# Suaiba/Mammo-CLIP-Dissect

Hardware: AMD Instinct MI355X
Metric: probe images/sec dissected (763 concepts, all layers) (higher is better)
Workload: dtype f32; 1 GPU; configs[1]: M-Mammo-CLIP Dissect through the drop-in driver describe_broad_neurons.main(): Mammo-CLIP ViT-B/16 target+dissector (random init), weak: 10000 images per GPU, synthetic 224x224 images resident in HBM, 763 concepts, 12 layers x 768 neurons, soft_wpmi top_k=100; CSV + args.txt + activation cache files written inside the step; entry_point=mammo_clip_dissect_amd.concept_vit.describe_broad_neurons.main, images_per_gpu=10000, global_images=10000, batch=2500, parallelism=image-sharded dp1, activation_cache_written=True

## Files before the change

### mammo-clip-dissect_amd/_lib.py

```python
import ctypes
import os

_HERE = os.path.dirname(os.path.abspath(__file__))
LIB_PATH = os.environ.get("MCD_LIB_PATH") or os.path.join(_HERE, "csrc", "libmcd_hip.so")

_i64 = ctypes.c_int64
_int = ctypes.c_int
_f = ctypes.c_float
_p = ctypes.c_void_p
_sz = ctypes.c_size_t

SIGNATURES = {
    "mcd_last_error": (ctypes.c_char_p, []),
    "mcd_abi_version": (_int, []),
    "mcd_normalize_rows": (_int, [_p, _i64, _i64, _i64, _p, _i64, _p]),
    "mcd_center_cube_normalize_rows": (_int, [_p, _i64, _i64, _i64, _f, _p, _i64, _p]),
    "mcd_prepare_rows_gathered": (_int, [_p, _i64, _i64, _int, ctypes.POINTER(_i64), _i64, _i64, _i64, _int, _f, _p, _i64,
                                         _p]),
    "mcd_embed_gemm_workspace": (_sz, [_i64, _i64, _i64, _int]),
    "mcd_embed_gemm": (_int, [_p, _i64, _p, _i64, _i64, _i64, _i64, _int, _p, _i64, _p, _sz, _p]),
    "mcd_embed_gemm_exp_workspace": (_sz, [_i64, _i64, _i64]),
    "mcd_embed_gemm_exp": (_int, [_p, _i64, _p, _i64, _i64, _i64, _i64, _f, _int, _p, _i64, _p, _p, _sz, _p]),
    "mcd_embed_gemm_exp_time_kernel": (_int, [_int]),
    "mcd_embed_gemm_exp_kernel_ms": (_f, []),
# ... 9 lines not shown
    "mcd_row_topk": (_int, [_p, _i64, _i64, _i64, _int, _p, _p, _p]),
    "mcd_hook_pool": (_int, [_p, _i64, _i64, _i64, _int, _p, _i64, _i64, _i64, _i64, _p]),
    "mcd_rank_reorder": (_int, [_p, _i64, _i64, _i64, _p, _p, _i64, _i64, _int, _p, _int, _f, _f, _p, _p, _i64, _p]),
    "mcd_vit_attention": (_int, [_p, _i64, _i64, _i64, _p, _p]),
    "mcd_vit_attention_long": (_int, [_p, _i64, _i64, _i64, _p, _p]),
    "mcd_vit_attention_cls": (_int, [_p, _i64, _p, _i64, _i64, _p, _i64, _i64, _i64, _i64, _i64, _p, _p]),
    "mcd_layer_norm": (_int, [_p, _i64, _i64, _p, _p, _f, _p, _p]),
    "mcd_patchify": (_int, [_p, _i64, _i64, _i64, _i64, _i64, _p, _p]),
    "mcd_conv_stem_nhwc": (_int, [_p, _i64, _i64, _i64, _i64, _p, _p, _i64, _p, _p]),
    "mcd_dwconv_bn_silu": (_int, [_p, _i64, _i64, _i64, _i64, _p, _p, _int, _int, _int, _p, _p, _i64, _p]),
    "mcd_se_gate": (_int, [_p, _i64, _i64, _i64, _i64, _p, _p, _i64, _p, _p, _p, _p]),
    "mcd_channel_scale": (_int, [_p, _i64, _i64, _i64, _p, _p]),
    "mcd_hook_pool_nhwc": (_int, [_p, _i64, _i64, _i64, _int, _p, _i64, _i64, _i64, _i64, _p]),
    "mcd_conv7x7s2_nhwc": (_int, [_p, _i64, _i64, _i64, _i64, _p, _i64, _p, _p]),
    "mcd_bn_relu_maxpool_nhwc": (_int, [_p, _i64, _i64, _i64, _i64, _p, _p, _p, _p]),
    "mcd_conv_igemm_nhwc": (_int, [_p, _i64, _i64, _i64, _i64, _p, _p, _i64, _int, _int, _int, _int, _p, _p]),
    "mcd_conv_igemm_res_nhwc": (_int, [_p, _i64, _i64, _i64, _i64, _p, _p, _p, _i64, _int, _int, _int, _int, _p, _p]),
    "mcd_conv3x3s2_nhwc": (_int, [_p, _i64, _i64, _i64, _i64, _p, _p, _i64, _int, _p, _p]),
    "mcd_avgpool2_nhwc": (_int, [_p, _i64, _i64, _i64, _i64, _p, _p]),
    "mcd_attnpool_tokens": (_int, [_p, _i64, _i64, _i64, _p, _p, _p]),
    "mcd_image_preprocess": (_int, [_p, _i64, _i64, _i64, _p, _i64, _i64, _p, _i64, _i64, _i64, _i64, _i64, _i64, _p, _p, _i64,
                                    _p]),
    "mcd_image_minmax_workspace": (_sz, [_i64, _i64, _i64, _i64]),
    "mcd_image_minmax_normalize": (_int, [_p, _i64, _i64, _i64, _i64, _int, _f, _f, _p, _i64, _p, _sz, _p]),
}
TEXT_SIGNATURES = {
    "mcd_vit_attention_keylen": (_int, [_p, _i64, _i64, _i64, _p, _p, _p]),
    "mcd_text_embed_ln": (_int, [_p, _p, _p, _p, _p, _p, _p, _f, _i64, _i64, _i64, _i64, _i64, _p, _p]),
}
CLIP_SIGNATURES = {
    "mcd_vit_attention_causal": (_int, [_p, _i64, _i64, _i64, _p, _p]),
    "mcd_quick_gelu": (_int, [_p, _i64, _p, _p]),
}
TOKEN_SIGNATURES = {
    "mcd_token_mean": (_int, [_p, _int, _int, _int, _i64, _i64, _int, _p, _i64, _p]),
}
SENTENCE_SIGNATURES = {
    "mcd_vit_attention_relbias": (_int, [_p, _i64, _i64, _i64, _p, _p, _p, _p]),
    "mcd_masked_mean_l2": (_int, [_p, _int, _int, _int, _p, _int, _p, _p]),
}
MASK_SIGNATURES = {
    "mcd_patchify_kept": (_int, [_p, _p, _i64, _i64, _i64, _i64, _i64, _i64, _p, _p]),
    "mcd_token_restore": (_int, [_p, _i64, _p, _p, _p, _i64, _i64, _i64, _i64, _p, _p]),
}
_pp = ctypes.POINTER(_p)
CACHE_SIGNATURES = {
    "mcd_hook_pool_rows": (_int, [_p, _i64, _i64, _i64, _int, _p, _i64, _i64, _i64, _i64, _p, _i64, _p]),
    "mcd_cache_stream_open": (_int, [_int, _pp, ctypes.POINTER(_i64), _p, _int, _sz, _pp]),
    "mcd_cache_stream_reserve": (_int, [_p, _int, _p]),
    "mcd_cache_stream_push": (_int, [_p, _int, _p, _i64, _i64, _p]),
    "mcd_cache_stream_close": (_int, [_p]),
    "mcd_cache_stream_abort": (_int, [_p]),
}

MCD_E_ARG = -1
MCD_E_RANGE = -2
MCD_E_WORKSPACE = -3
MCD_E_UNSUPPORTED = -5

_lib = None


class McdError(RuntimeError):

    def __init__(self, code, msg):
        super().__init__(msg)
        self.code = code


def load():
    global _lib
    if _lib is None:
        if not os.path.exists(LIB_PATH):
            raise ImportError(
                "mammo-clip-dissect_amd: %s not found. Build it with `python -c 'import __graft_entry__ as g; "
                "g.build()'` or `make -C mammo-clip-dissect_amd/csrc`. There is no CPU fallback." % LIB_PATH)
        L = ctypes.CDLL(LIB_PATH)
        for name, (res, args) in (list(SIGNATURES.items()) + list(TEXT_SIGNATURES.items()) + list(CLIP_SIGNATURES.items())
                                  + list(TOKEN_SIGNATURES.items()) + list(SENTENCE_SIGNATURES.items())
                                  + list(MASK_SIGNATURES.items()) + list(CACHE_SIGNATURES.items())):
            fn = getattr(L, name)
            fn.restype = res
            fn.argtypes = args
        _lib = L
    return _lib


def check(rc):
    if rc != 0:
        msg = load().mcd_last_error().decode("utf-8", "replace")
        raise McdError(rc, msg)


BLASLT_PATH = os.path.join(os.path.dirname(LIB_PATH), "libmcd_blaslt.so")
BLASLT_SIGNATURES = {
    "mcd_blaslt_last_error": (ctypes.c_char_p, []),
    "mcd_linear_residual_workspace": (_sz, []),
    "mcd_linear_residual": (_int, [_p, _i64, _p, _i64, _p, _p, _i64, _p, _i64, _i64, _i64, _i64, _p, _sz, _p]),
    "mcd_linear_residual_relu": (_int, [_p, _i64, _p, _i64, _p, _p, _i64, _p, _i64, _i64, _i64, _i64, _p, _sz, _p]),
    "mcd_linear_residual_plan_info": (_int, [_i64, _i64, _i64, ctypes.POINTER(_f), ctypes.POINTER(_int)]),
    "mcd_linear_residual_get_picks": (_int, [ctypes.POINTER(_i64), _int]),
    "mcd_linear_residual_set_pick": (_int, [_i64, _i64, _i64, _int, _int]),
}
_blaslt = None


def load_blaslt():
    global _blaslt
    if _blaslt is None:
        try:
            L = ctypes.CDLL(BLASLT_PATH)
            for name, (res, args) in BLASLT_SIGNATURES.items():
                fn = getattr(L, name)
                fn.restype = res
                fn.argtypes = args
            _blaslt = L
        except (OSError, AttributeError):
            _blaslt = False
    return _blaslt or None


HOST_PATH = os.path.join(_HERE, "csrc", "libmcd_host.so")
CACHE_HOST_SIGNATURES = {
    "mcd_zip_crc32": (ctypes.c_uint32, [ctypes.c_uint32, _p, _sz]),
    "mcd_cachefile_open": (_int, [ctypes.c_char_p, ctypes.c_char_p, _i64, _i64, _i64, _i64, _i64, _pp]),
    "mcd_cachefile_append": (_int, [_p, _p, _i64, _i64]),
    "mcd_cachefile_close": (_int, [_p]),
    "mcd_cachefile_abort": (None, [_p]),
    "mcd_cachefile_last_error": (ctypes.c_char_p, []),
}
_cache_host = None


# ... 22 lines not shown
```

### mammo-clip-dissect_amd/concept_vit/data_utils.py

```python
import collections
import math
import os
import unicodedata
import zlib

import torch
import torch.nn as nn
import torch.nn.functional as F
from torch.nn.modules import module as _nn_module

from .. import core

PROJ_DIM = 512
HIP_ATTENTION = os.environ.get("MCD_NO_HIP_ATTENTION", "0") != "1"
ATTENTION_EVENTS = None
_attention_calls = 0
FUSED_RESIDUAL = os.environ.get("MCD_NO_FUSED_RESIDUAL", "0") != "1"
CLS_ONLY_TAIL = os.environ.get("MCD_NO_CLS_ONLY_TAIL", "0") != "1"


HIP_LAYER_NORM = os.environ.get("MCD_NO_HIP_LAYER_NORM", "0") != "1"
HIP_MBCONV = os.environ.get("MCD_NO_HIP_MBCONV", "0") != "1"
HIP_RESNET = os.environ.get("MCD_NO_HIP_RESNET", "0") != "1"
HIP_CLIP_RN = os.environ.get("MCD_NO_HIP_CLIP_RN", "0") != "1"
HIP_TEXT = os.environ.get("MCD_NO_HIP_TEXT", "0") != "1"
HIP_CLIP_TEXT = os.environ.get("MCD_NO_HIP_CLIP_TEXT", "0") != "1"
MAX_BATCH = 65535


def _hip_eligible(on_gpu, dtype, grad):
    return bool(on_gpu) and dtype == torch.float32 and not grad


def _eligible(x):
    return isinstance(x, torch.Tensor) and _hip_eligible(x.is_cuda, x.dtype, torch.is_grad_enabled())


def _tower_gate(flag, module, x):
    return bool(flag and _eligible(x) and x.dim() == 4 and not module.training and x.shape[0] <= MAX_BATCH
                and core.linear_residual_available())


def _under_2g(*elements):
    return all(n * 4 < 2 ** 31 for n in elements)


class _LayerNorm(nn.LayerNorm):

    def forward(self, x):
        D = x.shape[-1]
        if (HIP_LAYER_NORM and _eligible(x) and x.is_contiguous() and len(self.normalized_shape) == 1 and D % 4 == 0
                and D <= 2048 and self.weight is not None and self.bias is not None):
            return core.layer_norm(x, self.weight, self.bias, self.eps)
        return super().forward(x)


def _linear(mod, x):
    if _fused_residual_ok(x) and x.is_contiguous() and mod.bias is not None:
        return core.linear_residual(None, x, mod.weight, mod.bias)
    return mod(x)


def _fused_residual_ok(x):
    return bool(FUSED_RESIDUAL and _eligible(x) and core.linear_residual_available())


def attention_route(T, D, heads, masked, on_gpu, dtype, needs_grad):
    if not (HIP_ATTENTION and not masked and _hip_eligible(on_gpu, dtype, needs_grad) and D == 64 * heads):
        return "sdpa"
    if T <= core.VIT_ATTENTION_MAX_T:
        return "k9"
    if T <= core.VIT_ATTENTION_LONG_MAX_T and _under_2g(T * 3 * D):
        return "long"
    return "sdpa"


def cls_tail_route(flag, fused_ok, masked, training, T, D, heads, depth, hooks_clear, last_hooks_token0):
    return bool(flag and HIP_ATTENTION and fused_ok and not masked and not training and D == 64 * heads
                and 1 <= T <= core.VIT_ATTENTION_CLS_MAX_T and depth >= 1 and hooks_clear and last_hooks_token0)


def embed_gate(P, H, W, table_rows):
    return bool(P >= 2 and P % 2 == 0 and H % P == 0 and W % P == 0 and 1 + (H // P) * (W // P) == table_rows)


def _token0_hooks(m):
    return all(getattr(h, "token0_only", False) for h in m._forward_hooks.values())


def _cls_tail_ok(x, blocks, container, clear=(), token0=()):
    if not (CLS_ONLY_TAIL and isinstance(x, torch.Tensor) and x.dim() == 3) or len(blocks) == 0:
        return False
    last = blocks[-1]
    hooks_clear = not (_nn_module._global_forward_hooks or _nn_module._global_forward_pre_hooks or last._forward_pre_hooks
                       or any(_hooked(c) for c in last.children()) or any(_hooked(m) for m in clear)
                       or container._forward_hooks or container._forward_pre_hooks)
    return cls_tail_route(CLS_ONLY_TAIL, _fused_residual_ok(x), False, container.training or last.training, x.shape[1],
                          x.shape[2], last.attn.heads, len(blocks), hooks_clear, all(_token0_hooks(m) for m in (last,) + token0))


def _class_pos_residual(pos, cls, bias, B):
    r = pos.detach().expand(B, -1, -1).contiguous()
    r[:, 0] = cls.detach() + pos.detach()[0] if bias is None else cls.detach() + pos.detach()[0] - bias.detach()
    return r


def _attend(qkv, heads, choice, arg=None):
    B, T, D = qkv.shape[0], qkv.shape[1], qkv.shape[2] // 3
    if choice == "k9":
        global _attention_calls
        _attention_calls += 1
        timed = ATTENTION_EVENTS is not None and _attention_calls % 8 == 0
        if timed:
            e0, e1 = torch.cuda.Event(enable_timing=True), torch.cuda.Event(enable_timing=True)
            e0.record()
        o = core.vit_attention(qkv, heads)
        if timed:
            e1.record()
            ATTENTION_EVENTS.append((e0, e1, B, T, heads))
        return o
    if choice == "long":
        return core.vit_attention_long(qkv, heads)
    if choice == "causal":
        return core.vit_attention_causal(qkv, heads)
    if choice == "keylen":
        return core.vit_attention_keylen(qkv, heads, arg)
    if choice == "relbias":
        return core.vit_attention_relbias(qkv, heads, *arg)
    q, k, v = qkv.view(B, T, 3, heads, D // heads).permute(2, 0, 3, 1, 4)
    o = F.scaled_dot_product_attention(q, k, v, attn_mask=arg)
    return o.transpose(1, 2).reshape(B, T, D)


def _attend_cls(q, kv):
    return core.vit_attention_cls(q, kv[:, :, 0], kv[:, :, 1])


_BlockOps = collections.namedtuple("_BlockOps", "ln1 ln2 qkv proj fc1 fc2 heads")


def _ln_ops(ln):
    return ln.weight, ln.bias, ln.eps


def _lin_ops(lin):
    return lin.weight, lin.bias


def _norm(x, ln, k10=True):
    return core.layer_norm(x, *ln) if k10 else F.layer_norm(x, x.shape[-1:], *ln)


def _gelu(h):
    return F.gelu(h)


def _quick_gelu_(h):
    return core.quick_gelu(h, out=h)


def _block_hip(p, x, attn, attn_arg=None, post=False, act=_gelu, cls_only=False, k10=True):
    B, T, D = x.shape
    x = x.contiguous()
    n = x if post else _norm(x, p.ln1, k10)
    w, b = p.qkv
    if cls_only:
        kv = core.linear_residual(None, n, w[D:], None if b is None else b[D:]).view(B, T, 2, p.heads, D // p.heads)
        o = _attend_cls(core.linear_residual(None, n[:, 0], w[:D], None if b is None else b[:D]), kv)
        x = x[:, 0]
    else:
        o = _attend(core.linear_residual(None, n, w, b), p.heads, attn, attn_arg).contiguous()
    x1 = core.linear_residual(x, o, *p.proj)
    if post:
        x1 = _norm(x1, p.ln1, k10)
    h = act(core.linear_residual(None, x1 if post else _norm(x1, p.ln2, k10), *p.fc1))
    if post:
        return _norm(core.linear_residual(x1, h, *p.fc2), p.ln2, k10)
    out = core.linear_residual(x1, h, *p.fc2, out=x1)
    return out.unsqueeze(1) if cls_only else out


class _Attention(nn.Module):
    def __init__(self, dim, heads):
        super().__init__()
        self.heads = heads
        self.qkv = nn.Linear(dim, 3 * dim)
        self.proj = nn.Linear(dim, dim)

    def forward(self, x, mask=None):
        return self.proj(self.heads_out(x, mask))

    def heads_out(self, x, mask=None):
        qkv = self.qkv(x)
        route = attention_route(x.shape[1], x.shape[2], self.heads, mask is not None, qkv.is_cuda, qkv.dtype,
                                torch.is_grad_enabled() and qkv.requires_grad)
        return _attend(qkv, self.heads, route, mask)


class _LayerScale(nn.Module):

    def __init__(self, dim, init):
        super().__init__()
        self.lambda1 = nn.Parameter(init * torch.ones(dim))

    def forward(self, x):
        return x * self.lambda1


_BLOCK_SKIPPED = ("norm1", "attn", "norm2", "fc1", "fc2", "layer_scale1", "layer_scale2")


class _Block(nn.Module):

    def __init__(self, dim, heads, mlp, eps=1e-12, layer_scale=None):
        super().__init__()
        self.norm1 = _LayerNorm(dim, eps=eps)
        self.attn = _Attention(dim, heads)
        self.norm2 = _LayerNorm(dim, eps=eps)
        self.fc1 = nn.Linear(dim, mlp)
        self.fc2 = nn.Linear(mlp, dim)
        self.scaled = layer_scale is not None
        if self.scaled:
            self.layer_scale1 = _LayerScale(dim, layer_scale)
            self.layer_scale2 = _LayerScale(dim, layer_scale)

    def forward(self, x, mask=None, cls_only=False):
        cls_only = cls_only and mask is None
        if cls_only or (_fused_residual_ok(x) and not _hooks_on(self, _BLOCK_SKIPPED)):
            B, T, D = x.shape
            route = attention_route(T, D, self.attn.heads, mask is not None, x.is_cuda, x.dtype, False)
            return _block_hip(self._ops(), x, route, mask, cls_only=cls_only, k10=HIP_LAYER_NORM and D % 4 == 0 and D <= 2048)
        if self.scaled:
            x = x + self.layer_scale1(self.attn(self.norm1(x), mask))
            return x + self.layer_scale2(self.fc2(F.gelu(self.fc1(self.norm2(x)))))
        x = x + self.attn(self.norm1(x), mask)
        return x + self.fc2(F.gelu(self.fc1(self.norm2(x))))

    def _ops(self):
        wp, bp, w2, b2 = self._residual_weights()
        return _BlockOps(_ln_ops(self.norm1), _ln_ops(self.norm2), _lin_ops(self.attn.qkv), (wp, bp), _lin_ops(self.fc1),
                         (w2, b2), self.attn.heads)

    def _residual_weights(self):
        a = self.attn
        if not self.scaled:
            return a.proj.weight, a.proj.bias, self.fc2.weight, self.fc2.bias

        def build(m):
            l1, l2 = m.layer_scale1.lambda1.detach(), m.layer_scale2.lambda1.detach()
            return ((l1[:, None] * m.attn.proj.weight.detach()).contiguous(), (l1 * m.attn.proj.bias.detach()).contiguous(),
                    (l2[:, None] * m.fc2.weight.detach()).contiguous(), (l2 * m.fc2.bias.detach()).contiguous())
        return _folded(self, ("layer_scale1", "layer_scale2", "attn", "fc2"), build)


class _Encoder(nn.Module):
    def __init__(self, depth, dim, heads, mlp, list_name, eps=1e-12, layer_scale=None):
        super().__init__()
        setattr(self, list_name, nn.ModuleList([_Block(dim, heads, mlp, eps, layer_scale) for _ in range(depth)]))
        self._list_name = list_name

    def forward(self, x, mask=None, cls_only=False):
        blocks = getattr(self, self._list_name)
        for i, blk in enumerate(blocks):
            x = blk(x, mask, cls_only=True) if cls_only and i == len(blocks) - 1 else blk(x, mask)
        return x


def image_hw(image_size):
    if isinstance(image_size, (tuple, list)):
        h, w = image_size
        return int(h), int(w)
    return int(image_size), int(image_size)


def _parse_hw(text):
    if text.isdigit():
        return int(text)
    h, sep, w = text.partition("x")
    if sep and h.isdigit() and w.isdigit():
        return int(h), int(w)
    return None


class ViTTower(nn.Module):

    def __init__(self, image_size=224, patch=16, dim=768, depth=12, heads=12, mlp=3072, list_name="layer", eps=1e-12,
                 layer_scale=None):
        super().__init__()
        self.out_dim = dim
        h, w = image_hw(image_size)
        self._build_embedding(dim, patch, (h // patch) * (w // patch))
        self.encoder = _Encoder(depth, dim, heads, mlp, list_name, eps, layer_scale)
        self.layernorm = _LayerNorm(dim, eps=eps)

# ... 1196 lines not shown
    ok = (flag and _hip_eligible(on_gpu, dtype, grad) and not training and D == 64 * heads and D % 4 == 0 and D <= 2048
          and 1 <= T <= core.VIT_ATTENTION_LONG_MAX_T and _under_2g(T * 3 * D) and 1 <= B <= MAX_BATCH and fused_ok)
    return "hip" if ok else "aten"


def quick_gelu(x):
    return x * torch.sigmoid(1.702 * x)


class _QuickGELU(nn.Module):
    def forward(self, x):
        return quick_gelu(x)


class _ClipMHA(nn.Module):

    def __init__(self, dim, heads):
        super().__init__()
        self.heads = heads
        self.in_proj_weight = nn.Parameter(torch.empty(3 * dim, dim))
        self.in_proj_bias = nn.Parameter(torch.zeros(3 * dim))
        self.out_proj = nn.Linear(dim, dim)

    def forward(self, x, causal=False):
        B, T, D = x.shape
        q, k, v = F.linear(x, self.in_proj_weight, self.in_proj_bias).view(B, T, 3, self.heads, D // self.heads).permute(2, 0, 3, 1, 4)
        o = F.scaled_dot_product_attention(q, k, v, is_causal=causal)
        return self.out_proj(o.transpose(1, 2).reshape(B, T, D))


class _ClipResBlock(nn.Module):

    def __init__(self, dim, heads, causal=False):
        super().__init__()
        self.causal = causal
        self.attn = _ClipMHA(dim, heads)
        self.ln_1 = nn.LayerNorm(dim)
        self.mlp = nn.Sequential()
        self.mlp.add_module("c_fc", nn.Linear(dim, 4 * dim))
        self.mlp.add_module("gelu", _QuickGELU())
        self.mlp.add_module("c_proj", nn.Linear(4 * dim, dim))
        self.ln_2 = nn.LayerNorm(dim)

    def forward(self, x, hip=False, cls_only=False):
        if hip and not _hooks_on(self, _CLIP_BLOCK_SKIPPED):
            attn = "causal" if self.causal else "k9" if x.shape[1] <= core.VIT_ATTENTION_MAX_T else "long"
            return _block_hip(self._ops(), x, attn, act=_quick_gelu_, cls_only=cls_only)
        x = x + self.attn(self.ln_1(x), self.causal)
        return x + self.mlp(self.ln_2(x))

    def _ops(self):
        a, m = self.attn, self.mlp
        return _BlockOps(_ln_ops(self.ln_1), _ln_ops(self.ln_2), (a.in_proj_weight, a.in_proj_bias), _lin_ops(a.out_proj),
                         _lin_ops(m.c_fc), _lin_ops(m.c_proj), a.heads)


class _ClipTransformer(nn.Module):
    def __init__(self, width, layers, heads, causal=False):
        super().__init__()
        self.width, self.layers = width, layers
        self.resblocks = nn.ModuleList([_ClipResBlock(width, heads, causal) for _ in range(layers)])

    def forward(self, x, hip=False, cls_only=False):
        for i, blk in enumerate(self.resblocks):
            x = blk(x, hip, cls_only and i == len(self.resblocks) - 1)
        return x


class _ClipVisionTransformer(nn.Module):

    def __init__(self, input_resolution, patch_size, width, layers, heads, output_dim):
        super().__init__()
        self.input_resolution, self.output_dim = input_resolution, output_dim
        self.conv1 = nn.Conv2d(3, width, patch_size, patch_size, bias=False)
        scale = width ** -0.5
        self.class_embedding = nn.Parameter(scale * torch.randn(width))
        self.positional_embedding = nn.Parameter(scale * torch.randn((input_resolution // patch_size) ** 2 + 1, width))
        self.ln_pre = nn.LayerNorm(width)
        self.transformer = _ClipTransformer(width, layers, heads)
        self.ln_post = nn.LayerNorm(width)
        self.proj = nn.Parameter(scale * torch.randn(width, output_dim))

    def route(self, x):
        P = self.conv1.kernel_size[0]
        n = self.positional_embedding.shape[0]
        heads = self.transformer.resblocks[0].attn.heads if len(self.transformer.resblocks) else 0
        if not (isinstance(x, torch.Tensor) and x.dim() == 4 and x.is_contiguous()
                and embed_gate(P, x.shape[2], x.shape[3], n)):
            return "aten"
        return clip_tower_route(HIP_CLIP_TEXT, x.is_cuda, x.dtype, torch.is_grad_enabled(), self.training, x.shape[0], n,
                                self.conv1.out_channels, heads, _fused_residual_ok(x))

    def forward(self, x):
        x = x.to(self.conv1.weight.dtype)
        if self.route(x) == "hip":
            return self._forward_hip(x)
        x = self.conv1(x).flatten(2).transpose(1, 2)
        x = torch.cat([self.class_embedding.expand(x.shape[0], 1, -1), x], dim=1) + self.positional_embedding
        x = self.transformer(self.ln_pre(x))
        return self.ln_post(x[:, 0]) @ self.proj

    def _forward_hip(self, x):
        B = x.shape[0]
        P = self.conv1.kernel_size[0]
        t = core.linear_residual(self._embed_residual(B), core.patchify(x, P), self.conv1.weight.view(self.conv1.out_channels, -1))
        if _hooked(self.ln_pre) or _nn_module._global_forward_hooks or _nn_module._global_forward_pre_hooks:
            t = self.ln_pre(t)
# ... 1517 lines not shown
```

### mammo-clip-dissect_amd/core.py

```python
import ctypes
import functools

import torch

from . import _lib
from ._lib import McdError, check

POOL_MODES = {"avg": 0, "max": 1, "cls": 2, "none": 3}
POOL_SILU_AVG = 4
GEMM_MODES = {"f32": 0, "bf16x3": 1, "bf16": 2}


def _stream():
    return ctypes.c_void_p(torch.cuda.current_stream().cuda_stream)


def _on_device(fn):
    @functools.wraps(fn)
    def wrapper(*args, **kw):
        dev = None
        for a in list(args) + list(kw.values()):
            if isinstance(a, torch.Tensor) and a.is_cuda:
                if dev is None:
                    dev = a.device
# ... 420 lines not shown
def quick_gelu(x, out=None):
    _need_gpu(x, out)
    if x.dtype != torch.float32 or not x.is_contiguous():
        raise TypeError("x must be a contiguous float32 tensor")
    if out is None:
        out = torch.empty_like(x)
    elif out.dtype != torch.float32 or out.shape != x.shape or not out.is_contiguous():
        raise TypeError("out must be a contiguous float32 tensor of x's shape")
    check(_lib.load().mcd_quick_gelu(x.data_ptr(), x.numel(), out.data_ptr(), _stream()))
    return out


@_on_device
def token_mean(x, t0=1, out=None):
    _need_gpu(x, out)
    if x.dtype != torch.float32 or x.dim() != 3 or x.stride(2) != 1:
        raise TypeError("x must be a float32 [B, T, D] tensor with a unit inner stride")
    B, T, D = x.shape
    if out is None:
        out = torch.empty((B, D), dtype=torch.float32, device=x.device)
    elif out.dtype != torch.float32 or tuple(out.shape) != (B, D) or out.stride(1) != 1:
        raise TypeError("out must be a float32 [B, D] tensor with a unit inner stride")
    check(_lib.load().mcd_token_mean(x.data_ptr(), B, T, D, x.stride(0), x.stride(1), t0, out.data_ptr(), out.stride(0),
                                     _stream()))
    return out


VIT_ATTENTION_CLS_MAX_T = 32768


@_on_device
def vit_attention_cls(q, k, v, out=None):
    _need_gpu(q, k, v, out)
    if any(t.dtype != torch.float32 for t in (q, k, v)) or k.dim() != 4 or k.shape[3] != 64 or v.shape != k.shape:
        raise TypeError("vit_attention_cls: float32 k and v of one shape [B, T, heads, 64]")
    B, T, H, _ = k.shape
    if q.dim() == 3:
        if tuple(q.shape) != (B, H, 64) or (H > 1 and q.stride(1) != 64):
            raise ValueError("vit_attention_cls: q must be [B, heads, 64] with a row's heads adjacent")
    elif tuple(q.shape) != (B, H * 64):
        raise ValueError("vit_attention_cls: q has shape %s, k %s" % (tuple(q.shape), tuple(k.shape)))
    if q.stride(-1) != 1 or any(t.stride(3) != 1 or (H > 1 and t.stride(2) != 64) for t in (k, v)):
        raise ValueError("vit_attention_cls: the heads*64 floats of a token must be adjacent in q, k and v")
    if out is None:
        out = torch.empty((B, H * 64), dtype=torch.float32, device=k.device)
    elif out.dtype != torch.float32 or tuple(out.shape) != (B, H * 64) or not out.is_contiguous():
        raise TypeError("out must be a contiguous float32 [B, heads*64] tensor")
    W = H * 64
    q_img = q.stride(0) if B > 1 else W
    row = [t.stride(1) if T > 1 else W for t in (k, v)]
    img = [t.stride(0) if B > 1 else max(T * r, W) for t, r in zip((k, v), row)]
    check(_lib.load().mcd_vit_attention_cls(q.data_ptr(), q_img, k.data_ptr(), row[0], img[0], v.data_ptr(), row[1], img[1],
                                            B, T, H, out.data_ptr(), _stream()))
    return out


@_on_device
def layer_norm(x, weight, bias, eps):
    _need_gpu(x, weight, bias)
    D = x.shape[-1]
    if x.dtype != torch.float32 or not x.is_contiguous() or weight.shape != (D,) or bias.shape != (D,):
        raise TypeError("layer_norm: contiguous float32 x and [D] weight / bias")
    y = torch.empty_like(x)
    L = _lib.load()
    check(L.mcd_layer_norm(x.data_ptr(), x.numel() // D, D, weight.data_ptr(), bias.data_ptr(), float(eps), y.data_ptr(),
                           _stream()))
    return y


@_on_device
def text_embed_ln(ids, type_ids, word, pos, type_table, weight, bias, eps, out=None):
    _need_gpu(word, pos, type_table, weight, bias, out)
    if ids.dim() != 2 or ids.dtype != torch.int64 or (type_ids is not None and (type_ids.dtype != torch.int64
                                                                               or type_ids.shape != ids.shape)):
        raise TypeError("text_embed_ln: ids (and type_ids) must be int64 [B, T]")
    B, T = ids.shape
    tables = (word, pos, type_table)
    if any(t.dtype != torch.float32 or t.dim() != 2 or not t.is_contiguous() for t in tables):
        raise TypeError("text_embed_ln: contiguous float32 [rows, D] tables")
    D = word.shape[1]
    if pos.shape[1] != D or type_table.shape[1] != D or weight.shape != (D,) or bias.shape != (D,):
        raise ValueError("text_embed_ln: the tables, weight and bias must share the width D=%d" % D)
    if T < 1 or T > pos.shape[0]:
        raise ValueError("text_embed_ln: T=%d tokens, the position table has %d rows" % (T, pos.shape[0]))
    for name, t, n in (("ids", ids, word.shape[0]), ("type_ids", type_ids, type_table.shape[0])):
        if t is not None and not t.is_cuda and t.numel() and (int(t.min()) < 0 or int(t.max()) >= n):
            raise ValueError("text_embed_ln: %s outside [0, %d)" % (name, n))
    ids = ids.to(word.device).contiguous()
    type_ids = None if type_ids is None else type_ids.to(word.device).contiguous()
    if out is None:
        out = torch.empty((B, T, D), dtype=torch.float32, device=word.device)
    elif out.dtype != torch.float32 or tuple(out.shape) != (B, T, D) or not out.is_contiguous():
        raise TypeError("out must be a contiguous float32 [B, T, D] tensor")
    check(_lib.load().mcd_text_embed_ln(ids.data_ptr(), None if type_ids is None else type_ids.data_ptr(), word.data_ptr(),
                                        pos.data_ptr(), type_table.data_ptr(), weight.data_ptr(), bias.data_ptr(), float(eps),
                                        B * T, T, D, word.shape[0], type_table.shape[0], out.data_ptr(), _stream()))
    return out


@_on_device
def patchify(x, patch):
    B, Cin, H, W = _nchw_image(x, "patchify: contiguous float32 [B, Cin, H, W]").shape
    if H % patch or W % patch:
        raise ValueError("patchify: %dx%d is not a multiple of the %d-pixel patch" % (H, W, patch))
    out = torch.empty((B, 1 + (H // patch) * (W // patch), Cin * patch * patch), dtype=torch.float32, device=x.device)
    L = _lib.load()
# ... 255 lines not shown
    if C % 4 or HW < 1:
        raise ValueError("attnpool_tokens: C = %d must be a multiple of 4 and the image non-empty" % C)
    if pos.dtype != torch.float32 or tuple(pos.shape) != (HW + 1, C) or not pos.is_contiguous():
        raise TypeError("attnpool_tokens: pos must be a contiguous float32 [%d, %d] tensor" % (HW + 1, C))
    _aligned16("attnpool_tokens: x and pos must be 16-byte aligned", x, pos)
    tok = torch.empty((B, HW + 1, C), dtype=torch.float32, device=x.device)
    L = _lib.load()
    check(L.mcd_attnpool_tokens(x.data_ptr(), B, HW, C, pos.data_ptr(), tok.data_ptr(), _stream()))
    return tok


_blaslt_ws = {}
LINEAR_EVENTS = None


def linear_residual_available():
    return _lib.load_blaslt() is not None


def encoder_gemm_picks():
    L = _lib.load_blaslt()
    if L is None:
        return []
    n = L.mcd_linear_residual_get_picks(None, 0)
    buf = (ctypes.c_int64 * (5 * max(n, 1)))()
    n = min(n, L.mcd_linear_residual_get_picks(buf, n))
    return [tuple(int(buf[5 * i + j]) for j in range(5)) for i in range(n)]


def set_encoder_gemm_picks(picks):
    L = _lib.load_blaslt()
    if L is None:
        return
    for M, N, K, has_res, pick in picks:
        L.mcd_linear_residual_set_pick(int(M), int(N), int(K), int(has_res), int(pick))


def _row_strided(t):
    return t.dim() == 2 and t.stride(1) == 1 and t.stride(0) >= t.shape[1]


@_on_device
def linear_residual(res, h, weight, bias=None, out=None, relu=False):
    L = _lib.load_blaslt()
    if L is None:
        raise ImportError("libmcd_blaslt.so is not available (make -C mammo-clip-dissect_amd/csrc)")
    _need_gpu(h, weight, bias, res, out)
    K = h.shape[-1]
    N = weight.shape[0]
    if weight.shape[1] != K or (res is not None and (res.shape[-1] != N or res.shape[:-1] != h.shape[:-1])):
        raise ValueError("linear_residual: shapes h %s, weight %s, res %s do not match"
                         % (tuple(h.shape), tuple(weight.shape), None if res is None else tuple(res.shape)))
    for t in (h, weight, bias, res, out):
        if t is not None and (t.dtype != torch.float32 or not (t.is_contiguous() or (t is h or t is res) and _row_strided(t))):
            raise TypeError("linear_residual: contiguous float32 tensors only (h and res: or 2-D row-strided)")
    M = h.numel() // K
    ldh = K if h.is_contiguous() else h.stride(0)
    ldr = N if res is None or res.is_contiguous() else res.stride(0)
    if out is None:
        out = torch.empty(h.shape[:-1] + (N,), dtype=torch.float32, device=h.device)
    elif tuple(out.shape) != tuple(h.shape[:-1]) + (N,):
        raise ValueError("linear_residual: out has shape %s" % (tuple(out.shape),))
    ws = _blaslt_ws.get(h.device)
    if ws is None:
        ws = _blaslt_ws[h.device] = torch.empty((L.mcd_linear_residual_workspace(),), dtype=torch.uint8, device=h.device)
    ev = LINEAR_EVENTS
    if ev is not None:
        e0, e1 = torch.cuda.Event(enable_timing=True), torch.cuda.Event(enable_timing=True)
        e0.record()
    fn = L.mcd_linear_residual_relu if relu else L.mcd_linear_residual
    rc = fn(h.data_ptr(), ldh, weight.data_ptr(), K, bias.data_ptr() if bias is not None else None,
            res.data_ptr() if res is not None else None, ldr, out.data_ptr(), N, M, N, K, ws.data_ptr(), ws.numel(), _stream())
    if ev is not None:
        e1.record()
        ev.append((e0, e1, M, N, K))
    if rc != 0:
        raise _lib.McdError(rc, L.mcd_blaslt_last_error().decode("utf-8", "replace"))
    return out


@_on_device
def hook_pool(x, mode, dst, row0, col0, neuron_major, rows=None):
    _need_gpu(x, dst)
    if rows is not None:
        _need_gpu(rows)
    if x.dtype != torch.float32:
        x = x.float()
    nhwc = mode in ("avg", "max") and channels_last(x, only=True)
    if not nhwc:
        x = x.contiguous()
    if x.dim() == 4:
        B, Cout, HW = x.shape[0], x.shape[1], x.shape[2] * x.shape[3]
        m = POOL_MODES[mode]
    elif x.dim() == 3:
        B, HW, Cout = x.shape
        m = POOL_MODES["cls"]
    elif x.dim() == 2:
        B, Cout = x.shape
        HW = 1
        m = POOL_MODES["none"]
    else:
        raise ValueError("unsupported hook output shape %s" % (tuple(x.shape),))
    if dst.dtype != torch.float32 or dst.dim() != 2 or dst.stride(1) != 1:
        raise TypeError("dst must be a 2-D float32 matrix with unit inner stride")
    need = (col0 + Cout, row0 + B) if neuron_major else (row0 + B, col0 + Cout)
    if row0 < 0 or col0 < 0 or dst.shape[0] < need[0] or dst.shape[1] < need[1]:
        raise IndexError("hook_pool: block [%d:%d, %d:%d] outside the activation matrix %s"
                         % (row0, row0 + B, col0, col0 + Cout, tuple(dst.shape)))
    if neuron_major:
        sn, su = 1, dst.stride(0)
    else:
        sn, su = dst.stride(0), 1
    if rows is not None and (rows.dtype != torch.float32 or rows.dim() != 2 or not rows.is_contiguous()
                             or rows.shape[0] < B or rows.shape[1] != Cout):
        raise TypeError("rows must be a contiguous float32 [>= %d, %d] block" % (B, Cout))
    L = _lib.load()
    if nhwc:
        check(L.mcd_hook_pool_nhwc(x.data_ptr(), B, Cout, HW, m, dst.data_ptr(), int(row0), int(col0), sn, su, _stream()))
        if rows is not None:
            if not neuron_major:
                raise TypeError("hook_pool: rows with a channels-last input needs a neuron-major dst")
            if B > 0:
                transpose(dst[col0:col0 + Cout, row0:row0 + B], out=rows[:B])
        return Cout
    if rows is not None:
# ... 256 lines not shown
```

Measured before the change: 4043 images/s.

## Fold key/value projections into the CLS query for the last-block attention

For the CLS-only tail block, the key weights are folded into the CLS query per head (u = q_h·Wk_h, pre-scaled for exp2). A new HIP kernel computes scores against the normalized tokens, applies softmax and mixes the tokens. The value projection is then applied only to the mixed per-head vectors. This avoids the full B×T K/V projection GEMM of the last layer. In exchange it adds per-head small GEMM launches and a cached folded-weight tensor, and linear_residual now accepts a row-strided output. The key bias is dropped, which is safe because softmax is shift-invariant.

```diff
diff --git a/include/mcd_clsfold.h b/include/mcd_clsfold.h
--- /dev/null
+++ b/include/mcd_clsfold.h
@@ -0,0 +1,18 @@
+#ifndef MCD_CLSFOLD_H
+#define MCD_CLSFOLD_H
+
+#include "mcd_hip.h"
+
+#ifdef __cplusplus
+extern "C" {
+#endif
+
+int mcd_cls_token_mix(const float* u, int64_t u_img, const float* n, int64_t n_row, int64_t n_img, int64_t B, int64_t T,
+                      int64_t H, int64_t D, float* m, int64_t m_img, mcd_stream_t stream);
+
+int64_t mcd_cls_token_mix_max_t(int64_t H, int64_t D);
+
+#ifdef __cplusplus
+}
+#endif
+#endif
diff --git a/mammo-clip-dissect_amd/_lib.py b/mammo-clip-dissect_amd/_lib.py
--- a/mammo-clip-dissect_amd/_lib.py
+++ b/mammo-clip-dissect_amd/_lib.py
@@ -85,6 +85,10 @@
     "mcd_cache_stream_close": (_int, [_p]),
     "mcd_cache_stream_abort": (_int, [_p]),
 }
+CLSFOLD_SIGNATURES = {
+    "mcd_cls_token_mix": (_int, [_p, _i64, _p, _i64, _i64, _i64, _i64, _i64, _i64, _p, _i64, _p]),
+    "mcd_cls_token_mix_max_t": (_i64, [_i64, _i64]),
+}
 
 MCD_E_ARG = -1
 MCD_E_RANGE = -2
@@ -111,7 +115,8 @@
         L = ctypes.CDLL(LIB_PATH)
         for name, (res, args) in (list(SIGNATURES.items()) + list(TEXT_SIGNATURES.items()) + list(CLIP_SIGNATURES.items())
                                   + list(TOKEN_SIGNATURES.items()) + list(SENTENCE_SIGNATURES.items())
-                                  + list(MASK_SIGNATURES.items()) + list(CACHE_SIGNATURES.items())):
+                                  + list(MASK_SIGNATURES.items()) + list(CACHE_SIGNATURES.items())
+                                  + list(CLSFOLD_SIGNATURES.items())):
             fn = getattr(L, name)
             fn.restype = res
             fn.argtypes = args
diff --git a/mammo-clip-dissect_amd/concept_vit/data_utils.py b/mammo-clip-dissect_amd/concept_vit/data_utils.py
--- a/mammo-clip-dissect_amd/concept_vit/data_utils.py
+++ b/mammo-clip-dissect_amd/concept_vit/data_utils.py
@@ -17,6 +17,8 @@
 _attention_calls = 0
 FUSED_RESIDUAL = os.environ.get("MCD_NO_FUSED_RESIDUAL", "0") != "1"
 CLS_ONLY_TAIL = os.environ.get("MCD_NO_CLS_ONLY_TAIL", "0") != "1"
+CLS_FOLD = os.environ.get("MCD_NO_CLS_FOLD", "0") != "1"
+CLS_FOLD_MIN_ROWS = 32768
 
 
 HIP_LAYER_NORM = os.environ.get("MCD_NO_HIP_LAYER_NORM", "0") != "1"
@@ -78,6 +80,11 @@
 def cls_tail_route(flag, fused_ok, masked, training, T, D, heads, depth, hooks_clear, last_hooks_token0):
     return bool(flag and HIP_ATTENTION and fused_ok and not masked and not training and D == 64 * heads
                 and 1 <= T <= core.VIT_ATTENTION_CLS_MAX_T and depth >= 1 and hooks_clear and last_hooks_token0)
+
+
+def cls_fold_route(flag, B, T, D, heads, min_rows):
+    return bool(flag and B * T >= min_rows and D == 64 * heads and D <= 2048 and 1 <= B <= core.CLS_TOKEN_MIX_MAX_B
+                and 1 <= T <= core.cls_token_mix_max_t(heads, D))
 
 
 def embed_gate(P, H, W, table_rows):
@@ -136,7 +143,26 @@
     return core.vit_attention_cls(q, kv[:, :, 0], kv[:, :, 1])
 
 
-_BlockOps = collections.namedtuple("_BlockOps", "ln1 ln2 qkv proj fc1 fc2 heads")
+_LOG2E = 1.4426950408889634
+
+
+def _attend_cls_folded(owner, qkv, heads, q, n):
+    w, b = qkv
+    B, T, D = n.shape
+    wkt = _folded(owner, (), lambda m: (w.detach()[D:2 * D].view(heads, 64, D).transpose(1, 2) * (_LOG2E / 8.0)).contiguous(),
+                  own=True)
+    u = torch.empty((B, heads, D), dtype=n.dtype, device=n.device)
+    for h in range(heads):
+        core.linear_residual(None, q[:, 64 * h:64 * h + 64], wkt[h], None, out=u[:, h])
+    m = core.cls_token_mix(u, n)
+    o = torch.empty((B, D), dtype=n.dtype, device=n.device)
+    for h in range(heads):
+        r = slice(2 * D + 64 * h, 2 * D + 64 * h + 64)
+        core.linear_residual(None, m[:, h], w[r], None if b is None else b[r], out=o[:, 64 * h:64 * h + 64])
+    return o
+
+
+_BlockOps = collections.namedtuple("_BlockOps", "ln1 ln2 qkv proj fc1 fc2 heads owner", defaults=(None,))
 
 
 def _ln_ops(ln):
@@ -164,7 +190,10 @@
     x = x.contiguous()
     n = x if post else _norm(x, p.ln1, k10)
     w, b = p.qkv
-    if cls_only:
+    if cls_only and p.owner is not None and cls_fold_route(CLS_FOLD, B, T, D, p.heads, CLS_FOLD_MIN_ROWS):
+        o = _attend_cls_folded(p.owner, p.qkv, p.heads, core.linear_residual(None, n[:, 0], w[:D], None if b is None else b[:D]), n)
+        x = x[:, 0]
+    elif cls_only:
         kv = core.linear_residual(None, n, w[D:], None if b is None else b[D:]).view(B, T, 2, p.heads, D // p.heads)
         o = _attend_cls(core.linear_residual(None, n[:, 0], w[:D], None if b is None else b[:D]), kv)
         x = x[:, 0]
@@ -239,7 +268,7 @@
     def _ops(self):
         wp, bp, w2, b2 = self._residual_weights()
         return _BlockOps(_ln_ops(self.norm1), _ln_ops(self.norm2), _lin_ops(self.attn.qkv), (wp, bp), _lin_ops(self.fc1),
-                         (w2, b2), self.attn.heads)
+                         (w2, b2), self.attn.heads, self.attn)
 
     def _residual_weights(self):
         a = self.attn
@@ -1542,7 +1571,7 @@
     def _ops(self):
         a, m = self.attn, self.mlp
         return _BlockOps(_ln_ops(self.ln_1), _ln_ops(self.ln_2), (a.in_proj_weight, a.in_proj_bias), _lin_ops(a.out_proj),
-                         _lin_ops(m.c_fc), _lin_ops(m.c_proj), a.heads)
+                         _lin_ops(m.c_fc), _lin_ops(m.c_proj), a.heads, a)
 
 
 class _ClipTransformer(nn.Module):
diff --git a/mammo-clip-dissect_amd/core.py b/mammo-clip-dissect_amd/core.py
--- a/mammo-clip-dissect_amd/core.py
+++ b/mammo-clip-dissect_amd/core.py
@@ -496,6 +496,37 @@
     img = [t.stride(0) if B > 1 else max(T * r, W) for t, r in zip((k, v), row)]
     check(_lib.load().mcd_vit_attention_cls(q.data_ptr(), q_img, k.data_ptr(), row[0], img[0], v.data_ptr(), row[1], img[1],
                                             B, T, H, out.data_ptr(), _stream()))
+    return out
+
+
+CLS_TOKEN_MIX_MAX_B = 65535
+
+
+def cls_token_mix_max_t(heads, D):
+    return int(_lib.load().mcd_cls_token_mix_max_t(int(heads), int(D)))
+
+
+@_on_device
+def cls_token_mix(u, n, out=None):
+    _need_gpu(u, n, out)
+    if u.dtype != torch.float32 or n.dtype != torch.float32 or u.dim() != 3 or n.dim() != 3:
+        raise TypeError("cls_token_mix: float32 u [B, heads, D] and n [B, T, D]")
+    B, H, D = u.shape
+    T = n.shape[1]
+    if n.shape[0] != B or n.shape[2] != D:
+        raise ValueError("cls_token_mix: u has shape %s, n %s" % (tuple(u.shape), tuple(n.shape)))
+    if u.stride(2) != 1 or n.stride(2) != 1 or (H > 1 and u.stride(1) != D):
+        raise ValueError("cls_token_mix: the D floats of a row, and the heads of an image in u, must be adjacent")
+    if out is None:
+        out = torch.empty((B, H, D), dtype=torch.float32, device=n.device)
+    elif (out.dtype != torch.float32 or tuple(out.shape) != (B, H, D) or out.stride(2) != 1
+          or (H > 1 and out.stride(1) != D)):
+        raise TypeError("out must be a float32 [B, heads, D] tensor with an image's heads*D floats adjacent")
+    u_img, m_img = (t.stride(0) if B > 1 else H * D for t in (u, out))
+    n_row = n.stride(1) if T > 1 else D
+    n_img = n.stride(0) if B > 1 else max(T * n_row, D)
+    check(_lib.load().mcd_cls_token_mix(u.data_ptr(), u_img, n.data_ptr(), n_row, n_img, B, T, H, D, out.data_ptr(), m_img,
+                                        _stream()))
     return out
 
 
@@ -857,11 +888,13 @@
         raise ValueError("linear_residual: shapes h %s, weight %s, res %s do not match"
                          % (tuple(h.shape), tuple(weight.shape), None if res is None else tuple(res.shape)))
     for t in (h, weight, bias, res, out):
-        if t is not None and (t.dtype != torch.float32 or not (t.is_contiguous() or (t is h or t is res) and _row_strided(t))):
-            raise TypeError("linear_residual: contiguous float32 tensors only (h and res: or 2-D row-strided)")
+        if t is not None and (t.dtype != torch.float32
+                              or not (t.is_contiguous() or (t is h or t is res or t is out) and _row_strided(t))):
+            raise TypeError("linear_residual: contiguous float32 tensors only (h, res and out: or 2-D row-strided)")
     M = h.numel() // K
     ldh = K if h.is_contiguous() else h.stride(0)
     ldr = N if res is None or res.is_contiguous() else res.stride(0)
+    ldo = N if out is None or out.is_contiguous() else out.stride(0)
     if out is None:
         out = torch.empty(h.shape[:-1] + (N,), dtype=torch.float32, device=h.device)
     elif tuple(out.shape) != tuple(h.shape[:-1]) + (N,):
@@ -875,7 +908,7 @@
         e0.record()
     fn = L.mcd_linear_residual_relu if relu else L.mcd_linear_residual
     rc = fn(h.data_ptr(), ldh, weight.data_ptr(), K, bias.data_ptr() if bias is not None else None,
-            res.data_ptr() if res is not None else None, ldr, out.data_ptr(), N, M, N, K, ws.data_ptr(), ws.numel(), _stream())
+            res.data_ptr() if res is not None else None, ldr, out.data_ptr(), ldo, M, N, K, ws.data_ptr(), ws.numel(), _stream())
     if ev is not None:
         e1.record()
         ev.append((e0, e1, M, N, K))
diff --git a/mammo-clip-dissect_amd/csrc/k_clsfold.hip b/mammo-clip-dissect_amd/csrc/k_clsfold.hip
--- /dev/null
+++ b/mammo-clip-dissect_amd/csrc/k_clsfold.hip
@@ -0,0 +1,203 @@
+#include "mcd_common.h"
+#include "../../include/mcd_clsfold.h"
+
+namespace {
+
+constexpr int CF_THREADS = 256;
+constexpr int CF_WAVES = CF_THREADS / 64;
+constexpr int CF_LDS_BYTES = 144 * 1024;
+constexpr int CF_MAX_D = 2048;
+constexpr int64_t CF_MAX_B = 65535;
+
+template <int CTRL>
+__device__ __forceinline__ float cf_dpp_add(float x) {
+    return x + __builtin_bit_cast(float, __builtin_amdgcn_update_dpp(0, __builtin_bit_cast(int, x), CTRL, 0xf, 0xf, true));
+}
+
+__device__ __forceinline__ float cf_row_sum(float x) {
+    x = cf_dpp_add<0xB1>(x);
+    x = cf_dpp_add<0x4E>(x);
+    x = cf_dpp_add<0x141>(x);
+    return cf_dpp_add<0x140>(x);
+}
+
+__device__ __forceinline__ float cf_dot4(float4 a, float4 b, float s) {
+    return fmaf(a.w, b.w, fmaf(a.z, b.z, fmaf(a.y, b.y, fmaf(a.x, b.x, s))));
+}
+
+template <int HC>
+__global__ __launch_bounds__(CF_THREADS) void cls_token_mix_kernel(const float* __restrict__ u, int64_t u_img,
+                                                                   const float* __restrict__ n, int64_t n_row, int64_t n_img,
+                                                                   int T, int H, int D, float* __restrict__ m, int64_t m_img) {
+    extern __shared__ __align__(16) float cf_lds[];
+    float* us = cf_lds;
+    float* sc = us + HC * D;
+    float* ls = sc + H * T;
+    const int tid = threadIdx.x, lane = tid & 63;
+    const int wave = __builtin_amdgcn_readfirstlane(tid >> 6);
+    const int sub = lane & 15, g = lane >> 4;
+    const int J = D >> 6, D4 = D >> 2;
+    const float* ub = u + (int64_t)blockIdx.x * u_img;
+    const float* nb = n + (int64_t)blockIdx.x * n_img;
+    float* mb = m + (int64_t)blockIdx.x * m_img;
+    const float4 zero = make_float4(0.f, 0.f, 0.f, 0.f);
+
+    for (int hb = 0; hb < H; hb += HC) {
+        if (hb) __syncthreads();
+        for (int i = tid; i < HC * D4; i += CF_THREADS)
+            reinterpret_cast<float4*>(us)[i] = reinterpret_cast<const float4*>(ub + (int64_t)hb * D)[i];
+        __syncthreads();
+        for (int t0 = wave * 4; t0 < T; t0 += 4 * CF_WAVES) {
+            const int t = t0 + g;
+            const bool ok = t < T;
+            const float* np = nb + (int64_t)(ok ? t : T - 1) * n_row + 4 * sub;
+            float s[HC];
+#pragma unroll
+            for (int i = 0; i < HC; ++i) s[i] = 0.f;
+            for (int j0 = 0; j0 < J; j0 += 4) {
+                float4 nv[4];
+#pragma unroll
+                for (int k = 0; k < 4; ++k) nv[k] = j0 + k < J ? *reinterpret_cast<const float4*>(np + 64 * (j0 + k)) : zero;
+#pragma unroll
+                for (int k = 0; k < 4; ++k) {
+                    if (j0 + k < J) {
+                        const float* up = us + 4 * sub + 64 * (j0 + k);
+#pragma unroll
+                        for (int i = 0; i < HC; ++i) s[i] = cf_dot4(nv[k], *reinterpret_cast<const float4*>(up + i * D), s[i]);
+                    }
+                }
+            }
+#pragma unroll
+            for (int i = 0; i < HC; ++i) {
+                const float r = cf_row_sum(s[i]);
+                if (ok && sub == 0) sc[(hb + i) * T + t] = r;
+            }
+        }
+    }
+    __syncthreads();
+
+    for (int h = wave; h < H; h += CF_WAVES) {
+        float* row = sc + h * T;
+        float mx = -INFINITY;
+        for (int t = lane; t < T; t += 64) mx = fmaxf(mx, row[t]);
+        mx = mcd_wave_max(mx);
+        float l = 0.f;
+        for (int t = lane; t < T; t += 64) {
+            const float p = __builtin_amdgcn_exp2f(row[t] - mx);
+            row[t] = p;
+            l += p;
+        }
+        l = mcd_wave_sum(l);
+        if (lane == 0) ls[h] = l;
+    }
+    __syncthreads();
+
+    for (int hb = 0; hb < H; hb += HC) {
+        const float* pr = sc + hb * T;
+        for (int c4 = tid; c4 < D4; c4 += CF_THREADS) {
+            const float* np = nb + 4 * c4;
+            float4 acc[HC];
+#pragma unroll
+            for (int i = 0; i < HC; ++i) acc[i] = zero;
+            int t = 0;
+            for (; t + 4 <= T; t += 4) {
+                float4 nv[4];
+#pragma unroll
+                for (int k = 0; k < 4; ++k) nv[k] = *reinterpret_cast<const float4*>(np + (int64_t)(t + k) * n_row);
+#pragma unroll
+                for (int k = 0; k < 4; ++k) {
+#pragma unroll
+                    for (int i = 0; i < HC; ++i) {
+                        const float p = pr[i * T + t + k];
+                        acc[i].x = fmaf(p, nv[k].x, acc[i].x);
+                        acc[i].y = fmaf(p, nv[k].y, acc[i].y);
+                        acc[i].z = fmaf(p, nv[k].z, acc[i].z);
+                        acc[i].w = fmaf(p, nv[k].w, acc[i].w);
+                    }
+                }
+            }
+            for (; t < T; ++t) {
+                const float4 v = *reinterpret_cast<const float4*>(np + (int64_t)t * n_row);
+#pragma unroll
+                for (int i = 0; i < HC; ++i) {
+                    const float p = pr[i * T + t];
+                    acc[i].x = fmaf(p, v.x, acc[i].x);
+                    acc[i].y = fmaf(p, v.y, acc[i].y);
+                    acc[i].z = fmaf(p, v.z, acc[i].z);
+                    acc[i].w = fmaf(p, v.w, acc[i].w);
+                }
+            }
+#pragma unroll
+            for (int i = 0; i < HC; ++i) {
+                const float l = ls[hb + i];
+                *reinterpret_cast<float4*>(mb + (int64_t)(hb + i) * D + 4 * c4) =
+                    make_float4(acc[i].x / l, acc[i].y / l, acc[i].z / l, acc[i].w / l);
+            }
+        }
+    }
+}
+
+bool cf_shape_ok(int64_t H, int64_t D) { return H >= 1 && D >= 1 && D <= CF_MAX_D && D % (64 * H) == 0; }
+
+size_t cf_lds_bytes(int64_t hc, int64_t T, int64_t H, int64_t D) { return (size_t)(hc * D + H * T + H) * sizeof(float); }
+
+int cf_heads_per_pass(int64_t T, int64_t H, int64_t D) {
+    for (int hc : {16, 12, 8, 4, 2})
+        if (H % hc == 0 && cf_lds_bytes(hc, T, H, D) <= (size_t)CF_LDS_BYTES) return hc;
+    return 1;
+}
+
+template <int HC>
+int cf_launch(const float* u, int64_t u_img, const float* n, int64_t n_row, int64_t n_img, int64_t B, int64_t T, int64_t H,
+              int64_t D, float* m, int64_t m_img, hipStream_t st) {
+    static bool attr_done[MCD_MAX_DEVICES] = {};
+    const int dev = mcd_cur_device();
+    if (!attr_done[dev]) {
+        if (hipFuncSetAttribute((const void*)cls_token_mix_kernel<HC>, hipFuncAttributeMaxDynamicSharedMemorySize,
+                                CF_LDS_BYTES) != hipSuccess)
+            return mcd_fail(MCD_E_LAUNCH, "mcd_cls_token_mix: cannot reserve %d bytes of LDS", CF_LDS_BYTES);
+        attr_done[dev] = true;
+    }
+    hipLaunchKernelGGL(cls_token_mix_kernel<HC>, dim3((unsigned)B), dim3(CF_THREADS), cf_lds_bytes(HC, T, H, D), st, u, u_img, n,
+                       n_row, n_img, (int)T, (int)H, (int)D, m, m_img);
+    MCD_LAUNCH_CHECK("cls_token_mix_kernel");
+    return MCD_OK;
+}
+
+}
+
+extern "C" int64_t mcd_cls_token_mix_max_t(int64_t H, int64_t D) {
+    if (!cf_shape_ok(H, D)) return 0;
+    return (CF_LDS_BYTES / (int64_t)sizeof(float) - D - H) / H;
+}
+
+extern "C" int mcd_cls_token_mix(const float* u, int64_t u_img, const float* n, int64_t n_row, int64_t n_img, int64_t B,
+                                 int64_t T, int64_t H, int64_t D, float* m, int64_t m_img, mcd_stream_t stream) {
+    MCD_REQUIRE(u && n && m, MCD_E_ARG, "mcd_cls_token_mix: NULL pointer");
+    MCD_REQUIRE(B >= 0 && H >= 1 && D >= 1, MCD_E_ARG, "mcd_cls_token_mix: bad shape B=%lld H=%lld D=%lld", (long long)B,
+                (long long)H, (long long)D);
+    MCD_REQUIRE(cf_shape_ok(H, D), MCD_E_UNSUPPORTED, "mcd_cls_token_mix: D=%lld must be a multiple of 64*H=%lld, at most %d",
+                (long long)D, (long long)(64 * H), CF_MAX_D);
+    MCD_REQUIRE(T >= 1 && T <= mcd_cls_token_mix_max_t(H, D), MCD_E_UNSUPPORTED,
+                "mcd_cls_token_mix: T=%lld tokens, between 1 and %lld for H=%lld D=%lld", (long long)T,
+                (long long)mcd_cls_token_mix_max_t(H, D), (long long)H, (long long)D);
+    MCD_REQUIRE(B <= CF_MAX_B, MCD_E_UNSUPPORTED, "mcd_cls_token_mix: B=%lld images, at most %lld", (long long)B,
+                (long long)CF_MAX_B);
+    MCD_REQUIRE(u_img >= H * D && m_img >= H * D && n_row >= D && n_img >= D, MCD_E_ARG,
+                "mcd_cls_token_mix: a stride (u_img=%lld n_row=%lld n_img=%lld m_img=%lld) is below its row: H*D=%lld, D=%lld",
+                (long long)u_img, (long long)n_row, (long long)n_img, (long long)m_img, (long long)(H * D), (long long)D);
+    MCD_REQUIRE(((uintptr_t)u | (uintptr_t)n | (uintptr_t)m) % 16 == 0 && (u_img | n_row | n_img | m_img) % 4 == 0, MCD_E_ARG,
+                "mcd_cls_token_mix: pointers must be 16-byte aligned and strides multiples of 4 floats");
+    if (B == 0) return MCD_OK;
+    hipStream_t st = (hipStream_t)stream;
+    switch (cf_heads_per_pass(T, H, D)) {
+#define MCD_CF(HC) case HC: return cf_launch<HC>(u, u_img, n, n_row, n_img, B, T, H, D, m, m_img, st)
+        MCD_CF(16);
+        MCD_CF(12);
+        MCD_CF(8);
+        MCD_CF(4);
+        MCD_CF(2);
+        default: MCD_CF(1);
+#undef MCD_CF
+    }
+}
```

Measured after the change: 4091 images/s, median of 6. +1.2%, better.
